# JakubValtar/basisu_rs

Measured on AMD Instinct MI355X. Metric: M 4x4 blocks/s UASTC->BC7 4096x4096, higher is better.
Workload: dtype u8

## Files before the change

### basisu_rs_amd/csrc/bu_hip.hip

```cpp
#include <hip/hip_runtime.h>

#include <stdio.h>
#include <stdlib.h>
#include <string.h>

#include <algorithm>
#include <array>
#include <atomic>
#include <chrono>
#include <future>
#include <iterator>
#include <mutex>
#include <new>
#include <thread>
#include <utility>
#include <vector>

#include "../../include/basisu_hip.h"
#include "bu_basis.hpp"
#include "bu_batch_plan.hpp"
#include "bu_uastc_dispatch.hpp"
#include "bu_etc1s_targets.hpp"
#include "bu_launch_plan.hpp"
#include "bu_rect_plan.hpp"

#include "bu_kernels.hpp"
#include "bu_etc1s_kernels.hpp"
#include "bu_context.hpp"
#include "bu_streams.hpp"
#include "bu_capi_slice.hpp"
#include "bu_capi_file.hpp"
#include "bu_capi_measure.hpp"
#include "bu_multi.hpp"
```

### basisu_rs_amd/csrc/bu_kernels.hpp

```cpp
#pragma once
namespace {

constexpr unsigned bu_lds_front(int target) { return target == 1 ? (unsigned)sizeof(BuBc7Tables) : 0u; }
constexpr unsigned bu_lds_table_bytes(int target) { return bu_lds_front(target) + bu_table_bytes(target); }
template <int WGS, int TARGET>
__device__ __forceinline__ void bu_stage_tables_n(uint4* dst, const BuTablesAll* __restrict__ src)
{
    constexpr BuTableRange R = bu_table_range(TARGET);
    constexpr int F = (int)bu_lds_front(TARGET) / 16;
    const uint4* s = reinterpret_cast<const uint4*>(TARGET == 1 ? reinterpret_cast<const void*>(src) : reinterpret_cast<const void*>(&src->t));
    uint4* d = dst;
    for (int i = threadIdx.x; i < F + (int)(R.hi / 16); i += WGS)
        if (i < F || i >= F + (int)(R.lo / 16)) d[i] = s[i];
    if constexpr (R.lo2 < R.hi2) {
        for (int i = F + R.lo2 / 16 + threadIdx.x; i < F + (int)(R.hi2 / 16); i += WGS) d[i] = s[i];
    }
}

__device__ __forceinline__ void bu_report(unsigned long long* status, unsigned long long block, int st)
{
    if (status) (void)__hip_atomic_fetch_min(status, (block << 8) | (unsigned long long)st, __ATOMIC_RELAXED, __HIP_MEMORY_SCOPE_SYSTEM);
}

typedef unsigned int bu_v4u __attribute__((ext_vector_type(4)));
typedef unsigned int bu_v2u __attribute__((ext_vector_type(2)));
__device__ __forceinline__ uint4 bu_ld_stream(const uint4* p)
{
    const bu_v4u r = __builtin_nontemporal_load(reinterpret_cast<const bu_v4u*>(p));
    return make_uint4(r.x, r.y, r.z, r.w);
}
__device__ __forceinline__ uint4 bu_ld_stream_global(const uint4* p)
{
    typedef const bu_v4u __attribute__((address_space(1))) * bu_global_v4u;
    const bu_v4u r = __builtin_nontemporal_load((bu_global_v4u)p);
    return make_uint4(r.x, r.y, r.z, r.w);
}
typedef bu_v4u __attribute__((address_space(1))) * bu_global_out_v4u;
typedef bu_v2u __attribute__((address_space(1))) * bu_global_out_v2u;
#ifndef BU_ST_MODE
#define BU_ST_MODE 4
#endif
#if BU_ST_MODE == 2
#define BU_ST_BITS " sc1"
#elif BU_ST_MODE == 3
#define BU_ST_BITS " sc0 sc1"
#elif BU_ST_MODE == 4
#define BU_ST_BITS " sc1 nt"
#endif
__device__ __forceinline__ void bu_st_stream(uint4* p, const uint4 v)
{
    bu_v4u r;
    r.x = v.x; r.y = v.y; r.z = v.z; r.w = v.w;
#if BU_ST_MODE == 0
    __builtin_nontemporal_store(r, (bu_global_out_v4u)p);
#elif BU_ST_MODE == 1
    *(bu_global_out_v4u)p = r;
#else
    asm volatile("global_store_dwordx4 %0, %1, off" BU_ST_BITS "\n\ts_nop 1" ::"v"(p), "v"(r) : "memory");
#endif
}
__device__ __forceinline__ void bu_st_stream(uint2* p, const uint2 v)
{
    bu_v2u r;
    r.x = v.x; r.y = v.y;
#if BU_ST_MODE == 1
    *(bu_global_out_v2u)p = r;
#else
    __builtin_nontemporal_store(r, (bu_global_out_v2u)p);
#endif
}

template <int TARGET>
__global__ __launch_bounds__(BU_WG) void bu_uastc_kernel(const uint4* __restrict__ in, void* __restrict__ out, size_t n_blocks,
                                                         unsigned bpr, unsigned long long base, unsigned long long* status,
                                                         const BuTablesAll* __restrict__ tables)
{
    __shared__ uint4 t_store[bu_lds_table_bytes(TARGET) / 16];
    BuTables& T = *reinterpret_cast<BuTables*>(t_store + bu_lds_front(TARGET) / 16);
    const size_t stride = (size_t)gridDim.x * BU_WG;
    size_t idx = (size_t)blockIdx.x * BU_WG + threadIdx.x;
    uint4 v = idx < n_blocks ? bu_ld_stream(in + idx) : make_uint4(0, 0, 0, 0);
    bu_stage_tables_n<BU_WG, TARGET>(t_store, tables);
    __syncthreads();
    while (idx < n_blocks) {
        const size_t next = idx + stride;
        const uint4 vn = next < n_blocks ? in[next] : make_uint4(0, 0, 0, 0);
        BuBlk b;
        b.w[0] = v.x;
        b.w[1] = v.y;
        b.w[2] = v.z;
        b.w[3] = v.w;
        const uint32_t mode = T.mode_lut[v.x & 127u];
        uint32_t o[TARGET == BU_TGT_RGBA ? 16 : 4];
#pragma unroll
        for (int i = 0; i < (TARGET == BU_TGT_RGBA ? 16 : 4); i++) o[i] = 0;
        const int st = bu_block_any<TARGET>(T, mode, b, o);
        if (st) {
            bu_report(status, base + idx, st);
#pragma unroll
            for (int i = 0; i < (TARGET == BU_TGT_RGBA ? 16 : 4); i++) o[i] = 0;
        }
        if constexpr (bu_out_words(TARGET) == 2) {
            reinterpret_cast<uint2*>(out)[idx] = make_uint2(o[0], o[1]);
        } else if constexpr (TARGET == BU_TGT_RGBA) {
            const size_t by = idx / bpr, bx = idx - by * bpr;
            uint4* img = reinterpret_cast<uint4*>(out);
#pragma unroll
            for (int r = 0; r < 4; r++) img[(4 * by + r) * (size_t)bpr + bx] = make_uint4(o[4 * r], o[4 * r + 1], o[4 * r + 2], o[4 * r + 3]);
        } else {
            reinterpret_cast<uint4*>(out)[idx] = make_uint4(o[0], o[1], o[2], o[3]);
        }
        v = vn;
        idx = next;
    }
}

__device__ __forceinline__ uint32_t bu_scan32(uint32_t v)
{
    v += (uint32_t)__builtin_amdgcn_update_dpp(0, (int)v, 0x111, 0xf, 0xf, false);
    v += (uint32_t)__builtin_amdgcn_update_dpp(0, (int)v, 0x112, 0xf, 0xf, false);
    v += (uint32_t)__builtin_amdgcn_update_dpp(0, (int)v, 0x114, 0xf, 0xf, false);
    v += (uint32_t)__builtin_amdgcn_update_dpp(0, (int)v, 0x118, 0xf, 0xf, false);
    v += (uint32_t)__builtin_amdgcn_update_dpp(0, (int)v, 0x142, 0xa, 0xf, false);
    return v;
}

struct BuRunDesc {
    const uint4* in;
    void* out;
    uint64_t base;
    uint32_t n;
    uint32_t vshift;
};
struct BuRunTable {
    BuRunDesc run[BU_MULTI_RUNS];
    uint32_t first_tile[BU_MULTI_RUNS + 32];
};
static_assert(sizeof(BuRunDesc) == 32 && sizeof(BuRunTable) <= 3968, "the run table must fit the 4 KiB of kernel arguments beside the other parameters");
struct BuTileDesc {
    const uint4* in;
    void* out;
    uint32_t first;
    uint32_t n;
    uint64_t base;
    uint32_t width;
};
enum { BU_LAYOUT_STRIP = 0, BU_LAYOUT_RECT = 1, BU_LAYOUT_MULTI = 2,
       BU_LAYOUT_MULTI_WHOLE = 3,
       BU_LAYOUT_RECTS = 4 };
constexpr unsigned BU_TICKET_STRIDE = 32, BU_TICKET_DONE = 8 * BU_TICKET_STRIDE, BU_TICKET_WORDS = 9 * BU_TICKET_STRIDE;
template <int TARGET, int WGS, int BPT, bool PREFETCH, int LAYOUT>
__device__ __forceinline__ void bu_uastc_sorted_body(const uint4* __restrict__ in, void* __restrict__ out, unsigned n_blocks,
                                                     unsigned bpr, unsigned long long base, unsigned long long* status,
                                                     const BuTablesAll* __restrict__ tables, unsigned cus, unsigned tile_rt,
                                                     const BuRunTable* __restrict__ runs, unsigned* __restrict__ ticket = nullptr,
                                                     const BuRectTable* __restrict__ rects = nullptr)
{
    if (cus != 0) {
        constexpr bool ROT = TARGET == BU_TGT_BC7 || TARGET == BU_TGT_ASTC;
        if (blockIdx.x >= 3 * cus) __builtin_amdgcn_s_setprio(ROT ? 1 : 3);
        else if (blockIdx.x >= 2 * cus) __builtin_amdgcn_s_setprio(2);
        else if (blockIdx.x >= cus) __builtin_amdgcn_s_setprio(ROT ? 3 : 1);
    }
    constexpr int BU_WG = WGS, BU_BPT = BPT, BU_TILE = WGS * BPT;
    __shared__ uint4 t_store[bu_lds_table_bytes(TARGET) / 16];
    BuTables& T = *reinterpret_cast<BuTables*>(t_store + bu_lds_front(TARGET) / 16);
    constexpr bool RECT = LAYOUT == BU_LAYOUT_RECT, MULTI = LAYOUT == BU_LAYOUT_MULTI || LAYOUT == BU_LAYOUT_MULTI_WHOLE;
    constexpr bool WHOLE = RECT || LAYOUT == BU_LAYOUT_MULTI_WHOLE;
    constexpr bool RECTS = LAYOUT == BU_LAYOUT_RECTS;
    static_assert(!RECTS || (BU_TILE == (int)BU_RECTS_TILE && PREFETCH), "the host numbers 1024-block tiles of rectangles; one compiled shape");
    constexpr uint32_t RECTS_ROW_BYTES = bu_rect_row_bytes(TARGET), RECTS_ROWS = bu_rect_rows_per_block(TARGET);
    constexpr bool BU_ALIAS = TARGET == BU_TGT_RGBA;
    static_assert(!BU_ALIAS || bu_lds_table_bytes(TARGET) + 4 * BU_TILE * 16 + BU_TILE + 1536 <= 80 * 1024,
                  "the RGBA32 workgroup no longer fits twice per CU: shrink BuTables or stage it per target in LDS too");
    __shared__ uint4 sblk_store[BU_ALIAS ? 1 : BU_TILE];
    __shared__ uint4 sout[BU_ALIAS ? 4 * BU_TILE : 1];
    uint4* const sblk = BU_ALIAS ? sout : sblk_store;
    constexpr bool INBLOCK = TARGET == BU_TGT_BC7 || TARGET == BU_TGT_ASTC;
    __shared__ uint8_t sst[INBLOCK ? 16 : BU_TILE];
    __shared__ uint32_t cnt[2][32], next_chunk[2];
    const unsigned tid = threadIdx.x, lane = tid & 63u;
    constexpr bool DYN_TILE = bu_dyn_tile(TARGET, BU_TILE) && LAYOUT != BU_LAYOUT_RECT;
    const unsigned tile_blocks = DYN_TILE ? tile_rt : (unsigned)BU_TILE;
    const unsigned n_tiles = (n_blocks + tile_blocks - 1) / tile_blocks;
    auto in_tile = [&](unsigned l) { return !DYN_TILE || l < tile_blocks; };
    static_assert(!RECT || BU_TILE % BU_RECT_W == 0, "rectangular tiles are BU_RECT_W blocks wide and of fixed size");
    const unsigned tpr = RECT ? bpr / BU_RECT_W : 1u;
    auto tile_xy = [&](unsigned t, unsigned& ty, unsigned& tx) {
        ty = (unsigned)(((unsigned long long)t * tile_rt) >> 32);
        tx = t - ty * tpr;
    };
    auto gidx = [&](unsigned t, unsigned l) {
        if constexpr (RECT) {
            unsigned ty, tx;
            tile_xy(t, ty, tx);
            return ((unsigned)(BU_TILE / BU_RECT_W) * ty + l / BU_RECT_W) * bpr + BU_RECT_W * tx + (l % BU_RECT_W);
        } else {
            return t * tile_blocks + l;
        }
    };
    auto has_block = [&](uint32_t k) { return WHOLE || k < 20u; };
    unsigned tile = blockIdx.x;
    __shared__ uint32_t s_next_tile[2];
    uint32_t my_draw = 0;
    unsigned* const my_counter = ticket ? ticket + (blockIdx.x & 7u) * BU_TICKET_STRIDE : nullptr;
    auto tile_of_draw = [&](uint32_t d) { return gridDim.x + 8u * d + (blockIdx.x & 7u); };
    if (ticket && tid == 0) my_draw = atomicAdd(my_counter, 1u);
    BuTileDesc td = {in, out, 0u, 0u, base, 0u}, tl = td;
    constexpr bool RUNS_IN_LDS = (MULTI || RECTS) && PREFETCH;
    __shared__ uint4 s_runs[RUNS_IN_LDS ? (RECTS ? sizeof(BuRectTable) : sizeof(BuRunTable)) / 16 : 1];
    const BuRunTable* R = runs;
    const BuRectTable* Q = rects;
    if constexpr (RUNS_IN_LDS && RECTS) {
        for (unsigned i = tid; i < sizeof(BuRectTable) / 16; i += WGS) s_runs[i] = reinterpret_cast<const uint4*>(rects)[i];
    } else if constexpr (RUNS_IN_LDS) {
        static_assert(sizeof(BuRunTable) % 16 == 0, "copied in 16-byte pieces");
        for (unsigned i = tid; i < sizeof(BuRunTable) / 16; i += WGS) s_runs[i] = reinterpret_cast<const uint4*>(runs)[i];
    }
    auto uni32 = [](uint32_t x) { return (uint32_t)__builtin_amdgcn_readfirstlane((int)x); };
    auto uni64 = [&](uint64_t x) { return (uint64_t)uni32((uint32_t)x) | ((uint64_t)uni32((uint32_t)(x >> 32)) << 32); };
    auto desc_of = [&](unsigned t, BuTileDesc& d) {
        if constexpr (MULTI) {
            if (t < n_tiles) {
                uint32_t r = 0;
#pragma unroll
                for (unsigned c = 0; c < BU_MULTI_RUNS + 32; c += 64) {
                    const uint32_t cnt = (uint32_t)__popcll(__ballot(R->first_tile[c + lane] <= t));
                    if (cnt) r = c + cnt - 1u;
                }
                r = (uint32_t)__builtin_amdgcn_readfirstlane((int)r);
                const BuRunDesc rv = R->run[r];
                const BuRunDesc rd = {reinterpret_cast<const uint4*>(uni64(reinterpret_cast<uint64_t>(rv.in))), reinterpret_cast<void*>(uni64(reinterpret_cast<uint64_t>(rv.out))),
                                      uni64(rv.base), uni32(rv.n), uni32(rv.vshift)};
                const uint32_t lt = t - uni32(R->first_tile[r]);
                if (rd.vshift != BU_RUN_STRIPS) {
                    const uint32_t ty = lt >> rd.vshift, tx = lt & ((1u << rd.vshift) - 1u), width = (uint32_t)BU_RECT_W << rd.vshift;
                    d = BuTileDesc{rd.in, rd.out, (uint32_t)(BU_TILE / BU_RECT_W) * ty * width + (uint32_t)BU_RECT_W * tx, (uint32_t)BU_TILE, rd.base, width};
                } else {
                    const uint32_t first = lt * (uint32_t)BU_TILE, left = rd.n - first;
                    d = BuTileDesc{rd.in, rd.out, first, left < (uint32_t)BU_TILE ? left : (uint32_t)BU_TILE, rd.base, 0u};
                }
            }
        }
    };
    BuRectTile qd = {}, ql = {};
    auto rect_of = [&](unsigned t, BuRectTile& d) {
        if constexpr (RECTS) {
            if (t < n_tiles) {
                static_assert(BU_RECT_JOBS == 64, "one first-tile number per lane");
                const uint32_t r = uni32((uint32_t)__popcll(__ballot(Q->first_tile[lane] <= t)) - 1u);
                const BuRectDesc jv = Q->job[r];
                const BuRectDesc jd = {uni64(jv.in), uni64(jv.out), uni64(jv.pitch), uni64(jv.base), uni32(jv.in_bpr), uni32(jv.w), uni32(jv.h), uni32(jv.tpr)};
                d = bu_rect_tile(jd, t - uni32(Q->first_tile[r]), RECTS_ROW_BYTES, RECTS_ROWS);
            }
        }
    };
    desc_of(tile, td);
    tl = td;
    rect_of(tile, qd);
    ql = qd;
    auto run_idx = [&](const BuTileDesc& d, unsigned l) { return d.first + ((WHOLE || d.width) ? (l / BU_RECT_W) * d.width + (l % BU_RECT_W) : l); };
    auto blk_src = [&](unsigned t, unsigned l) { return RECTS ? reinterpret_cast<const uint4*>(bu_rect_src(ql, l)) : MULTI ? tl.in + run_idx(tl, l) : in + gidx(t, l); };
    auto ld_blk = [&](unsigned t, unsigned l) { return (MULTI || RECTS) ? bu_ld_stream_global(blk_src(t, l)) : bu_ld_stream(blk_src(t, l)); };
    auto blk_valid = [&](unsigned t, unsigned l) {
        if constexpr (RECTS) return t < n_tiles && bu_rect_has(ql, l);
        else if constexpr (MULTI) return t < n_tiles && (WHOLE || l < tl.n);
        else return RECT ? t < n_tiles : (t < n_tiles && gidx(t, l) < n_blocks && in_tile(l));
    };
    constexpr BuTableRange TR = bu_table_range(TARGET);
    constexpr bool SPLIT = bu_lds_table_bytes(TARGET) > 16384;
    constexpr int TF = (int)bu_lds_front(TARGET) / 16, TV1 = (int)(TR.hi - TR.lo) / 16, TV2 = TR.lo2 < TR.hi2 ? (int)(TR.hi2 - TR.lo2) / 16 : 0;
    constexpr int TVT = TF + TV1 + TV2, TVN = (TVT + WGS - 1) / WGS;
    const uint4* const tsrc = reinterpret_cast<const uint4*>(TARGET == BU_TGT_BC7 ? reinterpret_cast<const void*>(tables) : reinterpret_cast<const void*>(&tables->t));
    auto tdst = [&](int i) { return i < TF ? i : (i < TF + TV1 ? (int)(TR.lo / 16) + i : TF + (int)(TR.lo2 / 16) + (i - TF - TV1)); };
    uint4 tv[TVN];
    if constexpr (!SPLIT) {
#pragma unroll
        for (int k = 0; k < TVN; k++) {
            const int i = k * WGS + (int)tid;
            tv[k] = i < TVT ? tsrc[tdst(i)] : make_uint4(0, 0, 0, 0);
        }
    }
    uint4 v[BU_BPT];
#pragma unroll
    for (int j = 0; j < BU_BPT; j++)
        v[j] = (RECT || blk_valid(tile, j * BU_WG + tid)) ? ld_blk(tile, j * BU_WG + tid) : make_uint4(0, 0, 0, 0);
    if constexpr (!SPLIT) {
#pragma unroll
        for (int k = 0; k < TVN; k++) {
            const int i = k * WGS + (int)tid;
            if (i < TVT) t_store[tdst(i)] = tv[k];
        }
    } else {
#pragma unroll
        for (int k = 0; k < TVN; k++) {
            const int i = k * WGS + (int)tid;
            tv[k] = i < TVT ? tsrc[tdst(i)] : make_uint4(0, 0, 0, 0);
        }
        static_assert(offsetof(BuTables, key_lut) % 4 == 0 && sizeof(T.key_lut[0]) == 128, "the target's key_lut is staged as 32 dwords");
        if (tid < 32) reinterpret_cast<uint32_t*>(T.key_lut[bu_cost_row(TARGET)])[tid] = reinterpret_cast<const uint32_t*>(tables->t.key_lut[bu_cost_row(TARGET)])[tid];
    }
    bool tables_staged = !SPLIT;
    if (tid < 64) (&cnt[0][0])[tid] = 0;
    if (tid < 2) next_chunk[tid] = 0;
    __syncthreads();
    if constexpr (RUNS_IN_LDS && RECTS) Q = reinterpret_cast<const BuRectTable*>(s_runs);
    else if constexpr (RUNS_IN_LDS) R = reinterpret_cast<const BuRunTable*>(s_runs);
    unsigned par = 0;
    unsigned next_of_loop = 0;
    constexpr bool STORES_LAST = PREFETCH && MULTI && (TARGET == BU_TGT_BC7 || (TARGET == BU_TGT_ASTC && WGS == 256 && WHOLE));
    auto key_of = [&](const BuTileDesc& d, unsigned l, uint32_t x) { return (WHOLE || l < d.n) ? (uint32_t)T.key_lut[bu_cost_row(TARGET)][x & 127u] : 31u; };
    uint32_t next_key[STORES_LAST ? BU_BPT : 1];
    uint32_t drawn_tile = 0;
    if constexpr (STORES_LAST) {
        if (tile < n_tiles) {
#pragma unroll
            for (int j = 0; j < BU_BPT; j++) next_key[j] = key_of(td, j * BU_WG + tid, v[j].x);
        }
        if (ticket && tid == 0) drawn_tile = tile_of_draw(my_draw);
        __builtin_amdgcn_s_waitcnt(0x0F70);
    }
    for (; tile < n_tiles; tile = next_of_loop, par ^= 1u) {
        [[maybe_unused]] const unsigned tbase = tile * tile_blocks;
        uint32_t key[BU_BPT], pos[BU_BPT];
        bool uniform = true;
#pragma unroll
        for (int j = 0; j < BU_BPT; j++) {
            if constexpr (STORES_LAST) {
                key[j] = next_key[j];
            } else {
                const bool valid = WHOLE || (RECTS ? bu_rect_has(qd, (unsigned)(j * BU_WG) + tid) : MULTI ? (unsigned)(j * BU_WG) + tid < td.n : (tbase + j * BU_WG + tid < n_blocks && in_tile(j * BU_WG + tid)));
                key[j] = valid ? T.key_lut[bu_cost_row(TARGET)][v[j].x & 127u] : 31u;
            }
            uniform = uniform && (__ballot(key[j] == (uint32_t)__builtin_amdgcn_readfirstlane(key[j])) == ~0ull) && has_block(key[j]);
        }
        if (uniform) {
            uint32_t lead[BU_BPT];
#pragma unroll
            for (int j = 0; j < BU_BPT; j++) lead[j] = lane == 0 ? atomicAdd(&cnt[par][key[j]], 64u) : 0u;
#pragma unroll
            for (int j = 0; j < BU_BPT; j++) pos[j] = (uint32_t)__builtin_amdgcn_readfirstlane(lead[j]) + lane;
        } else {
#pragma unroll
            for (int j = 0; j < BU_BPT; j++) pos[j] = atomicAdd(&cnt[par][key[j]], 1u);
        }
        if (ticket && tid == 0) s_next_tile[par] = STORES_LAST ? drawn_tile : tile_of_draw(my_draw);
        if (!tables_staged) {
#pragma unroll
            for (int k = 0; k < TVN; k++) {
                const int i = k * WGS + (int)tid;
                if (i < TVT) t_store[tdst(i)] = tv[k];
            }
            tables_staged = true;
        }
        __syncthreads();
        const uint32_t run_c = lane < 20u ? cnt[par][lane] : 0u;
        const uint32_t run_pk = run_c | (((run_c + 63u) >> 6) << 16);
        const uint32_t run_incl = bu_scan32(run_pk), run_excl = run_incl - run_pk;
        const uint32_t nc = (uint32_t)__builtin_amdgcn_readlane((int)run_incl, 31) >> 16;
        if (tid < 32) cnt[par ^ 1u][tid] = 0;
        if (tid == 0) next_chunk[par ^ 1u] = 0;
        uint32_t dest[BU_BPT];
#pragma unroll
        for (int j = 0; j < BU_BPT; j++) {
            const uint32_t st = (uint32_t)__builtin_amdgcn_ds_bpermute((int)(key[j] << 2), (int)run_excl) & 0xFFFFu;
            dest[j] = has_block(key[j]) ? st + pos[j] : 0u;
            if (has_block(key[j])) sblk[dest[j]] = v[j];
        }
        const unsigned ntile = ticket ? (unsigned)__builtin_amdgcn_readfirstlane((int)s_next_tile[par]) : tile + gridDim.x;
        next_of_loop = ntile;
        uint4 vn[BU_BPT];
        if constexpr (PREFETCH) {
            desc_of(ntile, tl);
            rect_of(ntile, ql);
#pragma unroll
            for (int j = 0; j < BU_BPT; j++) {
                vn[j] = blk_valid(ntile, j * BU_WG + tid) ? ld_blk(ntile, j * BU_WG + tid) : make_uint4(0, 0, 0, 0);
            }
        }
        if (ticket && tid == 0 && ntile < n_tiles) my_draw = atomicAdd(my_counter, 1u);
        __syncthreads();
        uint32_t c_next = 0;
        if (lane == 0) c_next = atomicAdd(&next_chunk[par], 1u);
        for (;;) {
            const uint32_t c = __builtin_amdgcn_readfirstlane(c_next);
            if (c >= nc) break;
            if (lane == 0) c_next = atomicAdd(&next_chunk[par], 1u);
            const uint32_t r = (uint32_t)__builtin_ctzll(__ballot((run_incl >> 16) > c));
            const uint32_t r_pk = (uint32_t)__builtin_amdgcn_readlane((int)run_pk, (int)r), r_ex = (uint32_t)__builtin_amdgcn_readlane((int)run_excl, (int)r);
            const uint32_t k64 = (c - (r_ex >> 16)) << 6;
            const uint32_t s0 = (r_ex & 0xFFFFu) + k64, left = (r_pk & 0xFFFFu) - k64, count = left < 64u ? left : 64u;
            const bool active = lane < count;
            const uint32_t slot = s0 + (active ? lane : 0u);
            const uint4 bv = sblk[slot];
            BuBlk b;
            b.w[0] = bv.x;
            b.w[1] = bv.y;
            b.w[2] = bv.z;
            b.w[3] = bv.w;
            constexpr int NO = TARGET == BU_TGT_RGBA ? 16 : 4;
            uint32_t o[NO];
#pragma unroll
            for (int i = 0; i < NO; i++) o[i] = 0;
            int st = BU_ST_BAD_MODE;
            if (active) {
                switch (r) {
#define BU_CASE(k) \
    case k: st = bu_block_mode<TARGET, BU_COST_ORDER[bu_cost_row(TARGET)][k]>(T, b, o); break;
                    BU_CASE(0) BU_CASE(1) BU_CASE(2) BU_CASE(3) BU_CASE(4) BU_CASE(5) BU_CASE(6) BU_CASE(7) BU_CASE(8) BU_CASE(9)
                    BU_CASE(10) BU_CASE(11) BU_CASE(12) BU_CASE(13) BU_CASE(14) BU_CASE(15) BU_CASE(16) BU_CASE(17) BU_CASE(18)
#undef BU_CASE
                default: break;
                }
                if constexpr (TARGET == BU_TGT_RGBA) {
#pragma unroll
                    for (int r2 = 0; r2 < 4; r2++) sout[r2 * BU_TILE + slot] = make_uint4(o[4 * r2], o[4 * r2 + 1], o[4 * r2 + 2], o[4 * r2 + 3]);
                    sst[slot] = (uint8_t)st;
                } else if constexpr (INBLOCK) {
                    sblk[slot] = make_uint4(o[0], o[1], o[2], o[3] | (uint32_t)st);
                } else {
                    sblk[slot] = make_uint4(o[0], o[1], o[2], o[3]);
                    sst[slot] = (uint8_t)st;
                }
            }
        }
        __syncthreads();
        if constexpr (STORES_LAST) {
            uint4 r[BU_BPT];
            bool has[BU_BPT];
            auto out_idx = [&](int j) { return run_idx(td, j * BU_WG + tid); };
#pragma unroll
            for (int j = 0; j < BU_BPT; j++) {
                has[j] = has_block(key[j]);
                if (has[j]) {
                    r[j] = sblk[dest[j]];
                    if ((r[j].x & 0xFFu) == 0u) {
                        bu_report(status, td.base + out_idx(j), (int)r[j].w);
                        r[j].w = 0;
                    }
                }
            }
#pragma unroll
            for (int j = 0; j < BU_BPT; j++) next_key[j] = key_of(tl, j * BU_WG + tid, vn[j].x);
            drawn_tile = tile_of_draw(my_draw);
            asm volatile("" : "+v"(drawn_tile));
#pragma unroll
            for (int j = 0; j < BU_BPT; j++)
                if (has[j]) bu_st_stream(reinterpret_cast<uint4*>(td.out) + out_idx(j), r[j]);
        } else {
#pragma unroll
        for (int j = 0; j < BU_BPT; j++) {
            if constexpr (RECTS) {
                if (has_block(key[j])) {
                    const unsigned l = j * BU_WG + tid;
                    const unsigned long long blk = qd.base + bu_rect_idx(qd, l);
                    const uint64_t dst = bu_rect_dst(qd, l, RECTS_ROW_BYTES, RECTS_ROWS);
                    if constexpr (INBLOCK) {
                        uint4 r = sblk[dest[j]];
                        if ((r.x & 0xFFu) == 0u) {
                            bu_report(status, blk, (int)r.w);
                            r.w = 0;
                        }
                        bu_st_stream(reinterpret_cast<uint4*>(dst), r);
                    } else {
                        const uint32_t st = sst[dest[j]];
                        if (st) bu_report(status, blk, (int)st);
                        if constexpr (TARGET == BU_TGT_RGBA) {
#pragma unroll
                            for (int r = 0; r < 4; r++) bu_st_stream(reinterpret_cast<uint4*>(dst + (uint64_t)r * qd.pitch), sout[r * BU_TILE + dest[j]]);
                        } else {
                            const uint4 r = sblk[dest[j]];
                            if constexpr (bu_out_words(TARGET) == 2) bu_st_stream(reinterpret_cast<uint2*>(dst), make_uint2(r.x, r.y));
                            else bu_st_stream(reinterpret_cast<uint4*>(dst), r);
                        }
                    }
                }
                continue;
            }
            if (has_block(key[j])) {
                const unsigned idx = MULTI ? run_idx(td, j * BU_WG + tid) : gidx(tile, j * BU_WG + tid);
                void* const out = td.out;
                const unsigned long long base = td.base;
                if constexpr (INBLOCK) {
                    uint4 r = sblk[dest[j]];
                    if ((r.x & 0xFFu) == 0u) {
                        bu_report(status, base + idx, (int)r.w);
                        r.w = 0;
                    }
                    bu_st_stream(reinterpret_cast<uint4*>(out) + idx, r);
                    continue;
                }
                const uint32_t st = sst[dest[j]];
                if (st) bu_report(status, base + idx, (int)st);
                if constexpr (TARGET == BU_TGT_RGBA) {
                    unsigned by, bx;
                    if constexpr (RECT) {
                        const unsigned l = j * BU_WG + tid;
                        unsigned ty, tx;
                        tile_xy(tile, ty, tx);
                        by = (unsigned)(BU_TILE / BU_RECT_W) * ty + l / BU_RECT_W;
                        bx = BU_RECT_W * tx + (l % BU_RECT_W);
                    } else {
                        by = idx / bpr;
                        bx = idx - by * bpr;
                    }
                    uint4* img = reinterpret_cast<uint4*>(out);
#pragma unroll
                    for (int r = 0; r < 4; r++) bu_st_stream(img + (size_t)((4 * by + r) * bpr + bx), sout[r * BU_TILE + dest[j]]);
                } else {
                    const uint4 r = sblk[dest[j]];
                    if constexpr (bu_out_words(TARGET) == 2) bu_st_stream(reinterpret_cast<uint2*>(out) + idx, make_uint2(r.x, r.y));
                    else bu_st_stream(reinterpret_cast<uint4*>(out) + idx, r);
                }
            }
        }
        }
        if constexpr (PREFETCH) {
#pragma unroll
            for (int j = 0; j < BU_BPT; j++) v[j] = vn[j];
            td = tl;
            qd = ql;
        } else {
            desc_of(ntile, tl);
            td = tl;
            rect_of(ntile, ql);
            qd = ql;
#pragma unroll
            for (int j = 0; j < BU_BPT; j++) v[j] = blk_valid(ntile, j * BU_WG + tid) ? ld_blk(ntile, j * BU_WG + tid) : make_uint4(0, 0, 0, 0);
        }
    }
    if (ticket && tid == 0) {
        if (atomicAdd(ticket + BU_TICKET_DONE, 1u) == gridDim.x - 1u) {
            for (unsigned k = 0; k < 8; k++) atomicExch(ticket + k * BU_TICKET_STRIDE, 0u);
            atomicExch(ticket + BU_TICKET_DONE, 0u);
        }
    }
}

template <int TARGET, int WGS, int BPT, int MINW, bool PREFETCH, int LAYOUT>
__global__ __launch_bounds__(WGS, MINW) void bu_uastc_sorted_kernel(const uint4* __restrict__ in, void* __restrict__ out, unsigned n_blocks,
                                                                unsigned bpr, unsigned long long base, unsigned long long* status,
                                                                const BuTablesAll* __restrict__ tables, unsigned cus, unsigned tile_rt,
                                                                unsigned* __restrict__ ticket)
{
    static_assert(LAYOUT != BU_LAYOUT_MULTI && LAYOUT != BU_LAYOUT_MULTI_WHOLE, "several runs per launch: bu_uastc_multi_kernel");
    bu_uastc_sorted_body<TARGET, WGS, BPT, PREFETCH, LAYOUT>(in, out, n_blocks, bpr, base, status, tables, cus, tile_rt, nullptr, ticket);
}

constexpr bool bu_multi_etc_2048(int target, int tile) { return bu_etc_family(target) && tile == 2048; }
template <int TARGET, int WGS, int BPT, bool PREFETCH = false, bool WHOLE = false>
__global__ __launch_bounds__(WGS, (TARGET == BU_TGT_ASTC && WGS == 512) ? 8 : bu_multi_etc_2048(TARGET, WGS * BPT) ? 4 : 1) void bu_uastc_multi_kernel(
    const BuRunTable table, unsigned n_tiles, unsigned bpr, unsigned long long* status, const BuTablesAll* __restrict__ tables, unsigned* __restrict__ ticket)
{
    static_assert(WGS * BPT == 1024 || bu_multi_etc_2048(TARGET, WGS * BPT), "the host numbers 1024-block tiles (ETC1 / ETC2 large batches: 2048-block ones)");
    static_assert(sizeof(BuRunTable) + 40 <= 4096, "the run table and the other arguments share the 4 KiB of kernel arguments");
    bu_uastc_sorted_body<TARGET, WGS, BPT, PREFETCH, WHOLE ? BU_LAYOUT_MULTI_WHOLE : BU_LAYOUT_MULTI>(nullptr, nullptr, n_tiles * (unsigned)(WGS * BPT), bpr, 0ull, status, tables, 0u,
                                                                                                        (unsigned)(WGS * BPT), &table, ticket);
}

template <int TARGET>
__global__ __launch_bounds__(512) void bu_uastc_rects_kernel(const BuRectTable table, unsigned n_tiles, unsigned long long* status, const BuTablesAll* __restrict__ tables)
{
    static_assert(sizeof(BuRectTable) + 24 <= 4096, "the job table and the other arguments share the 4 KiB of kernel arguments");
    bu_uastc_sorted_body<TARGET, 512, 2, true, BU_LAYOUT_RECTS>(nullptr, nullptr, n_tiles * BU_RECTS_TILE, 0u, 0ull, status, tables, 0u, BU_RECTS_TILE, nullptr, nullptr, &table);
}

__global__ void bu_status_reset_kernel(unsigned long long* words, unsigned n)
{
    for (unsigned i = threadIdx.x; i < n; i += blockDim.x) words[i] = ~0ull;
}

struct BuCrcTables {
    uint16_t t[4][256];
    uint16_t pw[256];
};
constexpr unsigned BU_CRC_PIECE = 65536;

__device__ __forceinline__ uint32_t bu_crc_gf_mul(uint32_t a, uint32_t b)
{
    uint32_t r = 0;
#pragma unroll
// ... 65 lines not shown
```

### basisu_rs_amd/csrc/bu_launch_plan.hpp

```cpp
#pragma once
#include <stddef.h>
#include <stdint.h>

#include <vector>

#include "bu_batch_plan.hpp"
#include "bu_uastc_dispatch.hpp"

constexpr int BU_WG = 256;
constexpr int BU_SORT_MIN_BLOCKS = 8;
constexpr bool bu_dyn_tile(int target, int tile) { return bu_etc_family(target) && tile == 4096; }
constexpr unsigned BU_RECT_W = 64;
constexpr unsigned BU_MULTI_RUNS = 96;
constexpr uint32_t BU_RUN_STRIPS = 0xFFFFFFFFu;
constexpr unsigned BU_TICKET_MIN_GRID = 8;

inline unsigned bu_grid_for(size_t n_blocks, unsigned cu_count)
{
    size_t wgs = (n_blocks + BU_WG - 1) / BU_WG;
    const size_t cap = (size_t)cu_count * 8;
    if (wgs > cap) wgs = cap;
    if (wgs == 0) wgs = 1;
    return (unsigned)wgs;
}

constexpr unsigned BU_ZEROCOPY_GRID = 64;

inline size_t bu_balanced_tile(size_t max_tile, size_t n_blocks, size_t slots, bool dynamic)
{
    if (!dynamic || slots == 0) return max_tile;
    const size_t per_slot = (n_blocks + slots - 1) / slots, rounds = (per_slot + max_tile - 1) / max_tile;
    size_t t = ((per_slot + rounds - 1) / rounds + 63) & ~(size_t)63;
    return t < 64 ? 64 : (t > max_tile ? max_tile : t);
}

struct BuShape {
    int wgs, bpt, minw;
    bool prefetch, rect;
    int per_cu;
    constexpr size_t tile() const { return (size_t)wgs * bpt; }
};
enum { BU_POLICY_EXCLUSIVE = 0, BU_POLICY_SHARED = 1, BU_POLICY_AUTO = 2,
       BU_POLICY_SHARED_FEW = 3 };
constexpr BuShape BuBigShape(int target, int policy)
{
    if (target == BU_TGT_BC7 || target == BU_TGT_ASTC)
        return policy == BU_POLICY_SHARED ? BuShape{256, 4, 1, true, true, 2}
                                          : BuShape{512, 2, target == BU_TGT_ASTC ? 8 : 1, true, true, 4};
    return policy == BU_POLICY_SHARED ? BuShape{512, 4, 4, target == BU_TGT_ETC1, true, 1} : BuShape{1024, 4, 1, true, true, 1};
}
constexpr bool bu_big_from_one_tile_per_cu(int target) { return target == BU_TGT_BC7 || target == BU_TGT_ASTC; }
constexpr BuShape BuOneTileShape(int target) { return BuShape{1024, 1, 1, false, target == BU_TGT_BC7 || target == BU_TGT_ASTC, 1}; }
constexpr BuShape BuEtcMidShape{512, 2, 1, false, false, 3};
constexpr BuShape BuZeroCopyShape{256, 4, 1, true, false, 1};
constexpr int BU_HOST_TILE = 1024;

struct BuSortedKey { int target, wgs, bpt, minw; bool prefetch, rect; };
constexpr BuSortedKey BU_SORTED_KERNELS[] = {
    {BU_TGT_BC7, 1024, 1, 1, false, false}, {BU_TGT_BC7, 1024, 1, 1, false, true}, {BU_TGT_BC7, 512, 2, 1, true, false}, {BU_TGT_BC7, 512, 2, 1, true, true},
    {BU_TGT_BC7, 256, 4, 1, true, false}, {BU_TGT_BC7, 256, 4, 1, true, true}, {BU_TGT_BC7, 512, 2, 1, false, false},
    {BU_TGT_ASTC, 1024, 1, 1, false, false}, {BU_TGT_ASTC, 1024, 1, 1, false, true}, {BU_TGT_ASTC, 512, 2, 8, true, false}, {BU_TGT_ASTC, 512, 2, 8, true, true},
    {BU_TGT_ASTC, 256, 4, 1, true, false}, {BU_TGT_ASTC, 256, 4, 1, true, true}, {BU_TGT_ASTC, 512, 2, 1, false, false},
    {BU_TGT_ETC1, 1024, 1, 1, false, false}, {BU_TGT_ETC1, 512, 2, 1, false, false}, {BU_TGT_ETC1, 1024, 4, 1, true, false}, {BU_TGT_ETC1, 1024, 4, 1, true, true},
    {BU_TGT_ETC1, 512, 4, 4, true, false}, {BU_TGT_ETC1, 512, 4, 4, true, true}, {BU_TGT_ETC1, 256, 4, 1, true, false}, {BU_TGT_ETC1, 256, 4, 1, true, true},
    {BU_TGT_ETC2, 1024, 1, 1, false, false}, {BU_TGT_ETC2, 512, 2, 1, false, false}, {BU_TGT_ETC2, 1024, 4, 1, true, false}, {BU_TGT_ETC2, 1024, 4, 1, true, true},
    {BU_TGT_ETC2, 512, 4, 4, false, false}, {BU_TGT_ETC2, 512, 4, 4, false, true}, {BU_TGT_ETC2, 256, 4, 1, true, false}, {BU_TGT_ETC2, 256, 4, 1, true, true},
    {BU_TGT_RGBA, 1024, 1, 1, true, false}, {BU_TGT_RGBA, 1024, 1, 1, true, true}, {BU_TGT_RGBA, 512, 2, 1, true, false}, {BU_TGT_RGBA, 512, 2, 1, true, true},
// ... 73 lines not shown
            const size_t slots = (size_t)cu_count * S.per_cu;
            const size_t tile_rt = bu_balanced_tile(S.tile(), nb, slots, bu_dyn_tile(target, (int)S.tile()));
            const size_t big_tiles = (nb + tile_rt - 1) / tile_rt;
            const unsigned cus = (priorities && (big_tiles <= slots || big_tiles % slots == 0)) ? cu_count : 0u;
            const bool ticket = priorities && bu_ticket_target(target) && big_tiles >= BU_TICKET_MIN_WALK * slots;
            go(S, big_tiles < slots ? big_tiles : slots, cus, tile_rt, ticket);
        };
        if (target == BU_TGT_RGBA) {
            const size_t cap = grid_cap ? (size_t)grid_cap : (size_t)cu_count * (policy == BU_POLICY_SHARED ? 1 : 2);
            const size_t grid = tiles < cap ? tiles : cap;
            const unsigned cus = (policy != BU_POLICY_SHARED && tiles >= 2 * grid) ? cu_count : 0u;
            const bool ticket = policy != BU_POLICY_SHARED && tiles >= BU_TICKET_MIN_WALK * grid;
            const bool wide = grid_cap == 0 && nb <= ((size_t)3 << 20);
            go(wide ? BuShape{1024, 1, 1, true, true, 2} : BuShape{512, 2, 1, true, true, 2}, grid, cus, BU_HOST_TILE, ticket);
        } else if (grid_cap) {
            go(BuZeroCopyShape, tiles < grid_cap ? tiles : grid_cap, cu_count, BuZeroCopyShape.tile(), false);
        } else if (nb <= (size_t)BU_HOST_TILE * cu_count) {
            go(BuOneTileShape(target), tiles, cu_count, BU_HOST_TILE, false);
        } else if (bu_big_from_one_tile_per_cu(target) || nb > (size_t)3 * BU_HOST_TILE * cu_count) {
            const BuShape shared = BuBigShape(target, BU_POLICY_SHARED);
            if (etc && nb >= ((size_t)1 << 20))
                go(shared, (nb + shared.tile() - 1) / shared.tile(), 0u, shared.tile(), false);
            else if (policy == BU_POLICY_SHARED_FEW && bu_big_from_one_tile_per_cu(target))
                go_big(BuShape{shared.wgs, shared.bpt, shared.minw, shared.prefetch, shared.rect, 4}, false);
            else if (policy == BU_POLICY_SHARED || policy == BU_POLICY_SHARED_FEW) go_big(shared, false);
            else if (target == BU_TGT_ASTC && nb >= ((size_t)1 << 21))
                go_big(BuShape{256, 4, 1, true, true, 5}, true);
            else go_big(BuBigShape(target, BU_POLICY_EXCLUSIVE), true);
        } else {
            go(BuEtcMidShape, tiles, cu_count, BU_HOST_TILE, false);
        }
    }
}

struct BuRunEntry { size_t run, offset, n; uint32_t vshift, first_tile; };
enum { BU_MULTI_ETC_2048 = 0, BU_MULTI_ONE_TILE = 1, BU_MULTI_WHOLE = 2, BU_MULTI_PERSIST = 3 };
struct BuRunsLaunch {
    size_t plain_run = SIZE_MAX;
    BuRunEntry entries[BU_MULTI_RUNS];
    size_t k = 0, n_tiles = 0;
    unsigned tile = 1024;
    bool all_whole = true;
    bool needs_policy = false;
    int kernel = BU_MULTI_PERSIST;
    unsigned grid = 0, block = 0;
    bool wants_ticket = false;
};

inline void bu_plan_runs(int kernel_target, const BuRun* runs, size_t n_runs, size_t blocks_per_row, unsigned cu_count, std::vector<BuRunsLaunch>& out)
{
    const int target = bu_shape_target(kernel_target);
    out.clear();
    const bool rect_target = target == BU_TGT_BC7 || target == BU_TGT_ASTC || target == BU_TGT_RGBA;
    const size_t real = (blocks_per_row >= 128 && (blocks_per_row & (blocks_per_row - 1)) == 0 && blocks_per_row <= ((size_t)1 << 20)) ? blocks_per_row : 0;
    const size_t virt = target == BU_TGT_RGBA ? 0 : 1;
    const size_t pitches[5] = {real, virt * 1024, virt * 2048, virt * 512, virt * 256};
    auto shift_of = [](size_t v) {
        uint32_t sh = 0;
        while (((size_t)BU_RECT_W << sh) < v) sh++;
        return sh;
    };
    for (size_t r0 = 0; r0 < n_runs;) {
        BuRunsLaunch l;
        if (target == BU_TGT_ETC1 || target == BU_TGT_ETC2) {
            size_t total = 0, tiles2 = 0;
            for (size_t i = r0; i < n_runs && i < r0 + BU_MULTI_RUNS; i++) {
                total += runs[i].n;
                tiles2 += (runs[i].n + 2047) / 2048;
            }
            if (total >= ((size_t)1 << 20) && tiles2 * 2048 <= total + total / 8) l.tile = 2048;
        }
        auto emit = [&](size_t run, size_t offset, size_t n, uint32_t vshift) {
            l.all_whole = l.all_whole && vshift != BU_RUN_STRIPS;
            l.entries[l.k++] = BuRunEntry{run, offset, n, vshift, (uint32_t)l.n_tiles};
            l.n_tiles += (n + l.tile - 1) / l.tile;
        };
        size_t used = 0;
        for (; r0 + used < n_runs && l.k < BU_MULTI_RUNS; used++) {
            const size_t ri = r0 + used, n = runs[ri].n;
            const size_t t = (n + l.tile - 1) / l.tile;
            if (l.n_tiles + t + 1 >= (((size_t)1 << 32) / l.tile)) break;
            size_t whole_pitch = 0, prefix_pitch = 0;
            if (rect_target) {
                for (const size_t v : pitches)
                    if (v && n % (16 * v) == 0) {
                        whole_pitch = v;
                        break;
                    }
                if (!whole_pitch && target == BU_TGT_RGBA && l.k + 2 <= BU_MULTI_RUNS)
                    for (const size_t v : pitches)
                        if (v && n >= 8 * 16 * v) {
                            prefix_pitch = v;
                            break;
                        }
            }
            if (whole_pitch) {
                emit(ri, 0, n, shift_of(whole_pitch));
            } else if (prefix_pitch) {
                const size_t prefix = n / (16 * prefix_pitch) * (16 * prefix_pitch);
                emit(ri, 0, prefix, shift_of(prefix_pitch));
                emit(ri, prefix, n - prefix, BU_RUN_STRIPS);
            } else {
                emit(ri, 0, n, BU_RUN_STRIPS);
            }
        }
        if (used <= 1) {
            out.emplace_back().plain_run = r0++;
            continue;
        }
        l.needs_policy = !(l.tile == 1024 && l.n_tiles <= (size_t)cu_count);
        out.push_back(l);
        r0 += used;
    }
}

// ... 15 lines not shown
```

Measured before the change: 189,800.

## Cache run lookup and precompute 32-bit lane offsets in multi-run kernel

The multi-run kernel now keeps a cursor on the current run and skips the ballot search over the run table when the next tile falls in the same run. Per-lane byte offsets are computed once per tile width and reused. Loads and stores use a uniform 64-bit base plus a 32-bit per-lane offset, so the store can use the SGPR-base addressing form. This is meant to cut per-tile descriptor work and per-block 64-bit address arithmetic, at the cost of more registers and a new constraint that offsets fit in 32 bits (large RGBA pitches fall back to plain runs).

```diff
diff --git a/basisu_rs_amd/csrc/bu_hip.hip b/basisu_rs_amd/csrc/bu_hip.hip
--- a/basisu_rs_amd/csrc/bu_hip.hip
+++ b/basisu_rs_amd/csrc/bu_hip.hip
@@ -23,6 +23,7 @@
 #include "bu_etc1s_targets.hpp"
 #include "bu_launch_plan.hpp"
 #include "bu_rect_plan.hpp"
+#include "bu_multi_addr.hpp"
 
 #include "bu_kernels.hpp"
 #include "bu_etc1s_kernels.hpp"
diff --git a/basisu_rs_amd/csrc/bu_kernels.hpp b/basisu_rs_amd/csrc/bu_kernels.hpp
--- a/basisu_rs_amd/csrc/bu_kernels.hpp
+++ b/basisu_rs_amd/csrc/bu_kernels.hpp
@@ -33,6 +33,13 @@
 {
     typedef const bu_v4u __attribute__((address_space(1))) * bu_global_v4u;
     const bu_v4u r = __builtin_nontemporal_load((bu_global_v4u)p);
+    return make_uint4(r.x, r.y, r.z, r.w);
+}
+typedef const char __attribute__((address_space(1))) * bu_global_bytes;
+__device__ __forceinline__ uint4 bu_ld_stream_global(uint64_t base, uint32_t off)
+{
+    typedef const bu_v4u __attribute__((address_space(1))) * bu_global_v4u;
+    const bu_v4u r = __builtin_nontemporal_load((bu_global_v4u)((bu_global_bytes)base + off));
     return make_uint4(r.x, r.y, r.z, r.w);
 }
 typedef bu_v4u __attribute__((address_space(1))) * bu_global_out_v4u;
@@ -67,6 +74,29 @@
     *(bu_global_out_v2u)p = r;
 #else
     __builtin_nontemporal_store(r, (bu_global_out_v2u)p);
+#endif
+}
+typedef char __attribute__((address_space(1))) * bu_global_out_bytes;
+__device__ __forceinline__ void bu_st_stream(uint64_t base, uint32_t off, const uint4 v)
+{
+    bu_v4u r;
+    r.x = v.x; r.y = v.y; r.z = v.z; r.w = v.w;
+#if BU_ST_MODE == 0
+    __builtin_nontemporal_store(r, (bu_global_out_v4u)((bu_global_out_bytes)base + off));
+#elif BU_ST_MODE == 1
+    *(bu_global_out_v4u)((bu_global_out_bytes)base + off) = r;
+#else
+    asm volatile("global_store_dwordx4 %0, %1, %2" BU_ST_BITS "\n\ts_nop 1" ::"v"(off), "v"(r), "s"(base) : "memory");
+#endif
+}
+__device__ __forceinline__ void bu_st_stream(uint64_t base, uint32_t off, const uint2 v)
+{
+    bu_v2u r;
+    r.x = v.x; r.y = v.y;
+#if BU_ST_MODE == 1
+    *(bu_global_out_v2u)((bu_global_out_bytes)base + off) = r;
+#else
+    __builtin_nontemporal_store(r, (bu_global_out_v2u)((bu_global_out_bytes)base + off));
 #endif
 }
 
@@ -145,6 +175,19 @@
     uint64_t base;
     uint32_t width;
 };
+template <bool MULTI, int BPT>
+struct BuMultiWalk {
+    BuMultiTile d = {}, l = {};
+    uint32_t off[BPT] = {};
+    uint32_t off_width = 0xFFFFFFFFu;
+    BuRunCursor cur = bu_no_run();
+};
+template <int BPT>
+struct BuMultiWalk<false, BPT> {};
+template <int BPT>
+__device__ __forceinline__ uint32_t bu_walk_n(const BuMultiWalk<true, BPT>& w) { return w.d.n; }
+template <int BPT>
+__device__ __forceinline__ uint32_t bu_walk_n(const BuMultiWalk<false, BPT>&) { return 0u; }
 enum { BU_LAYOUT_STRIP = 0, BU_LAYOUT_RECT = 1, BU_LAYOUT_MULTI = 2,
        BU_LAYOUT_MULTI_WHOLE = 3,
        BU_LAYOUT_RECTS = 4 };
@@ -207,6 +250,8 @@
     auto tile_of_draw = [&](uint32_t d) { return gridDim.x + 8u * d + (blockIdx.x & 7u); };
     if (ticket && tid == 0) my_draw = atomicAdd(my_counter, 1u);
     BuTileDesc td = {in, out, 0u, 0u, base, 0u}, tl = td;
+    BuMultiWalk<MULTI, BPT> mw;
+    constexpr uint32_t OUT_BYTES = TARGET == BU_TGT_RGBA ? 16u : (uint32_t)bu_out_words(TARGET) * 4u;
     constexpr bool RUNS_IN_LDS = (MULTI || RECTS) && PREFETCH;
     __shared__ uint4 s_runs[RUNS_IN_LDS ? (RECTS ? sizeof(BuRectTable) : sizeof(BuRunTable)) / 16 : 1];
     const BuRunTable* R = runs;
@@ -219,26 +264,28 @@
     }
     auto uni32 = [](uint32_t x) { return (uint32_t)__builtin_amdgcn_readfirstlane((int)x); };
     auto uni64 = [&](uint64_t x) { return (uint64_t)uni32((uint32_t)x) | ((uint64_t)uni32((uint32_t)(x >> 32)) << 32); };
-    auto desc_of = [&](unsigned t, BuTileDesc& d) {
+    auto desc_of = [&](unsigned t, BuMultiTile& d) {
         if constexpr (MULTI) {
             if (t < n_tiles) {
-                uint32_t r = 0;
-#pragma unroll
-                for (unsigned c = 0; c < BU_MULTI_RUNS + 32; c += 64) {
-                    const uint32_t cnt = (uint32_t)__popcll(__ballot(R->first_tile[c + lane] <= t));
-                    if (cnt) r = c + cnt - 1u;
-                }
-                r = (uint32_t)__builtin_amdgcn_readfirstlane((int)r);
-                const BuRunDesc rv = R->run[r];
-                const BuRunDesc rd = {reinterpret_cast<const uint4*>(uni64(reinterpret_cast<uint64_t>(rv.in))), reinterpret_cast<void*>(uni64(reinterpret_cast<uint64_t>(rv.out))),
-                                      uni64(rv.base), uni32(rv.n), uni32(rv.vshift)};
-                const uint32_t lt = t - uni32(R->first_tile[r]);
-                if (rd.vshift != BU_RUN_STRIPS) {
-                    const uint32_t ty = lt >> rd.vshift, tx = lt & ((1u << rd.vshift) - 1u), width = (uint32_t)BU_RECT_W << rd.vshift;
-                    d = BuTileDesc{rd.in, rd.out, (uint32_t)(BU_TILE / BU_RECT_W) * ty * width + (uint32_t)BU_RECT_W * tx, (uint32_t)BU_TILE, rd.base, width};
-                } else {
-                    const uint32_t first = lt * (uint32_t)BU_TILE, left = rd.n - first;
-                    d = BuTileDesc{rd.in, rd.out, first, left < (uint32_t)BU_TILE ? left : (uint32_t)BU_TILE, rd.base, 0u};
+                if (!bu_cursor_holds(mw.cur, t)) {
+                    uint32_t r = 0;
+                    uint32_t ln = lane;
+                    asm volatile("" : "+v"(ln));
+#pragma unroll
+                    for (unsigned c = 0; c < BU_MULTI_RUNS + 32; c += 64) {
+                        const uint32_t cnt = (uint32_t)__popcll(__ballot(R->first_tile[c + ln] <= t));
+                        if (cnt) r = c + cnt - 1u;
+                    }
+                    r = (uint32_t)__builtin_amdgcn_readfirstlane((int)r);
+                    const BuRunDesc rv = R->run[r];
+                    const BuRunRec rd = {uni64(reinterpret_cast<uint64_t>(rv.in)), uni64(reinterpret_cast<uint64_t>(rv.out)), uni64(rv.base), uni32(rv.n), uni32(rv.vshift)};
+                    mw.cur = bu_run_cursor(rd, uni32(R->first_tile[r]), (uint32_t)BU_TILE);
+                }
+                d = bu_tile_of(mw.cur, t, (uint32_t)BU_TILE, OUT_BYTES, TARGET == BU_TGT_RGBA ? bpr : 0u);
+                if (d.width != mw.off_width) {
+                    mw.off_width = d.width;
+#pragma unroll
+                    for (int j = 0; j < BPT; j++) mw.off[j] = bu_lane_off(WHOLE, d.width, (unsigned)(j * WGS) + tid);
                 }
             }
         }
@@ -255,16 +302,30 @@
             }
         }
     };
-    desc_of(tile, td);
+    if constexpr (MULTI) desc_of(tile, mw.d);
+    if constexpr (MULTI) mw.l = mw.d;
     tl = td;
     rect_of(tile, qd);
     ql = qd;
-    auto run_idx = [&](const BuTileDesc& d, unsigned l) { return d.first + ((WHOLE || d.width) ? (l / BU_RECT_W) * d.width + (l % BU_RECT_W) : l); };
-    auto blk_src = [&](unsigned t, unsigned l) { return RECTS ? reinterpret_cast<const uint4*>(bu_rect_src(ql, l)) : MULTI ? tl.in + run_idx(tl, l) : in + gidx(t, l); };
-    auto ld_blk = [&](unsigned t, unsigned l) { return (MULTI || RECTS) ? bu_ld_stream_global(blk_src(t, l)) : bu_ld_stream(blk_src(t, l)); };
+    auto blk_src = [&](unsigned t, unsigned l) { return RECTS ? reinterpret_cast<const uint4*>(bu_rect_src(ql, l)) : in + gidx(t, l); };
+    auto ld_one = [&](unsigned t, unsigned l) { return RECTS ? bu_ld_stream_global(blk_src(t, l)) : bu_ld_stream(blk_src(t, l)); };
+    auto ld_blk = [&](unsigned t, unsigned l, int j) {
+        if constexpr (MULTI) return bu_ld_stream_global(mw.l.in, mw.off[j]);
+        else return ld_one(t, l);
+    };
+    auto store_offsets = [&](uint32_t (&so)[MULTI ? BPT : 1]) {
+        if constexpr (MULTI) {
+#pragma unroll
+            for (int j = 0; j < BPT; j++) so[j] = mw.off[j];
+            if (mw.d.width != mw.off_width) {
+#pragma unroll
+                for (int j = 0; j < BPT; j++) so[j] = bu_lane_off(WHOLE, mw.d.width, (unsigned)(j * WGS) + tid);
+            }
+        }
+    };
     auto blk_valid = [&](unsigned t, unsigned l) {
         if constexpr (RECTS) return t < n_tiles && bu_rect_has(ql, l);
-        else if constexpr (MULTI) return t < n_tiles && (WHOLE || l < tl.n);
+        else if constexpr (MULTI) return t < n_tiles && (WHOLE || l < mw.l.n);
         else return RECT ? t < n_tiles : (t < n_tiles && gidx(t, l) < n_blocks && in_tile(l));
     };
     constexpr BuTableRange TR = bu_table_range(TARGET);
@@ -284,7 +345,7 @@
     uint4 v[BU_BPT];
 #pragma unroll
     for (int j = 0; j < BU_BPT; j++)
-        v[j] = (RECT || blk_valid(tile, j * BU_WG + tid)) ? ld_blk(tile, j * BU_WG + tid) : make_uint4(0, 0, 0, 0);
+        v[j] = (RECT || blk_valid(tile, j * BU_WG + tid)) ? ld_blk(tile, j * BU_WG + tid, j) : make_uint4(0, 0, 0, 0);
     if constexpr (!SPLIT) {
 #pragma unroll
         for (int k = 0; k < TVN; k++) {
@@ -309,13 +370,13 @@
     unsigned par = 0;
     unsigned next_of_loop = 0;
     constexpr bool STORES_LAST = PREFETCH && MULTI && (TARGET == BU_TGT_BC7 || (TARGET == BU_TGT_ASTC && WGS == 256 && WHOLE));
-    auto key_of = [&](const BuTileDesc& d, unsigned l, uint32_t x) { return (WHOLE || l < d.n) ? (uint32_t)T.key_lut[bu_cost_row(TARGET)][x & 127u] : 31u; };
+    auto key_of = [&](const BuMultiTile& d, unsigned l, uint32_t x) { return (WHOLE || l < d.n) ? (uint32_t)T.key_lut[bu_cost_row(TARGET)][x & 127u] : 31u; };
     uint32_t next_key[STORES_LAST ? BU_BPT : 1];
     uint32_t drawn_tile = 0;
     if constexpr (STORES_LAST) {
         if (tile < n_tiles) {
 #pragma unroll
-            for (int j = 0; j < BU_BPT; j++) next_key[j] = key_of(td, j * BU_WG + tid, v[j].x);
+            for (int j = 0; j < BU_BPT; j++) next_key[j] = key_of(mw.d, j * BU_WG + tid, v[j].x);
         }
         if (ticket && tid == 0) drawn_tile = tile_of_draw(my_draw);
         __builtin_amdgcn_s_waitcnt(0x0F70);
@@ -329,7 +390,7 @@
             if constexpr (STORES_LAST) {
                 key[j] = next_key[j];
             } else {
-                const bool valid = WHOLE || (RECTS ? bu_rect_has(qd, (unsigned)(j * BU_WG) + tid) : MULTI ? (unsigned)(j * BU_WG) + tid < td.n : (tbase + j * BU_WG + tid < n_blocks && in_tile(j * BU_WG + tid)));
+                const bool valid = WHOLE || (RECTS ? bu_rect_has(qd, (unsigned)(j * BU_WG) + tid) : MULTI ? (unsigned)(j * BU_WG) + tid < bu_walk_n(mw) : (tbase + j * BU_WG + tid < n_blocks && in_tile(j * BU_WG + tid)));
                 key[j] = valid ? T.key_lut[bu_cost_row(TARGET)][v[j].x & 127u] : 31u;
             }
             uniform = uniform && (__ballot(key[j] == (uint32_t)__builtin_amdgcn_readfirstlane(key[j])) == ~0ull) && has_block(key[j]);
@@ -371,11 +432,21 @@
         next_of_loop = ntile;
         uint4 vn[BU_BPT];
         if constexpr (PREFETCH) {
-            desc_of(ntile, tl);
+            if constexpr (MULTI) desc_of(ntile, mw.l);
             rect_of(ntile, ql);
-#pragma unroll
-            for (int j = 0; j < BU_BPT; j++) {
-                vn[j] = blk_valid(ntile, j * BU_WG + tid) ? ld_blk(ntile, j * BU_WG + tid) : make_uint4(0, 0, 0, 0);
+            if constexpr (MULTI && WHOLE) {
+                if (ntile < n_tiles) {
+#pragma unroll
+                    for (int j = 0; j < BU_BPT; j++) vn[j] = ld_blk(ntile, j * BU_WG + tid, j);
+                } else {
+#pragma unroll
+                    for (int j = 0; j < BU_BPT; j++) vn[j] = make_uint4(0, 0, 0, 0);
+                }
+            } else {
+#pragma unroll
+                for (int j = 0; j < BU_BPT; j++) {
+                    vn[j] = blk_valid(ntile, j * BU_WG + tid) ? ld_blk(ntile, j * BU_WG + tid, j) : make_uint4(0, 0, 0, 0);
+                }
             }
         }
         if (ticket && tid == 0 && ntile < n_tiles) my_draw = atomicAdd(my_counter, 1u);
@@ -428,26 +499,29 @@
         if constexpr (STORES_LAST) {
             uint4 r[BU_BPT];
             bool has[BU_BPT];
-            auto out_idx = [&](int j) { return run_idx(td, j * BU_WG + tid); };
+            uint32_t so[BU_BPT];
+            store_offsets(so);
 #pragma unroll
             for (int j = 0; j < BU_BPT; j++) {
                 has[j] = has_block(key[j]);
                 if (has[j]) {
                     r[j] = sblk[dest[j]];
                     if ((r[j].x & 0xFFu) == 0u) {
-                        bu_report(status, td.base + out_idx(j), (int)r[j].w);
+                        bu_report(status, mw.d.base + bu_lane_block(mw.d, so[j]), (int)r[j].w);
                         r[j].w = 0;
                     }
                 }
             }
 #pragma unroll
-            for (int j = 0; j < BU_BPT; j++) next_key[j] = key_of(tl, j * BU_WG + tid, vn[j].x);
+            for (int j = 0; j < BU_BPT; j++) next_key[j] = key_of(mw.l, j * BU_WG + tid, vn[j].x);
             drawn_tile = tile_of_draw(my_draw);
             asm volatile("" : "+v"(drawn_tile));
 #pragma unroll
             for (int j = 0; j < BU_BPT; j++)
-                if (has[j]) bu_st_stream(reinterpret_cast<uint4*>(td.out) + out_idx(j), r[j]);
+                if (has[j]) bu_st_stream(mw.d.out, so[j], r[j]);
         } else {
+        [[maybe_unused]] uint32_t so[MULTI ? BU_BPT : 1];
+        store_offsets(so);
 #pragma unroll
         for (int j = 0; j < BU_BPT; j++) {
             if constexpr (RECTS) {
@@ -477,8 +551,34 @@
                 }
                 continue;
             }
+            if constexpr (MULTI) {
+                if (has_block(key[j])) {
+                    const uint32_t lo = so[j];
+                    if constexpr (INBLOCK) {
+                        uint4 r = sblk[dest[j]];
+                        if ((r.x & 0xFFu) == 0u) {
+                            bu_report(status, mw.d.base + bu_lane_block(mw.d, lo), (int)r.w);
+                            r.w = 0;
+                        }
+                        bu_st_stream(mw.d.out, lo, r);
+                    } else {
+                        const uint32_t st = sst[dest[j]];
+                        if (st) bu_report(status, mw.d.base + bu_lane_block(mw.d, lo), (int)st);
+                        if constexpr (TARGET == BU_TGT_RGBA) {
+                            const uint32_t row0 = bu_lane_off_rgba(mw.d, lo, bpr);
+#pragma unroll
+                            for (int r = 0; r < 4; r++) bu_st_stream(mw.d.out, row0 + (uint32_t)r * bpr * 16u, sout[r * BU_TILE + dest[j]]);
+                        } else {
+                            const uint4 r = sblk[dest[j]];
+                            if constexpr (bu_out_words(TARGET) == 2) bu_st_stream(mw.d.out, lo >> 1, make_uint2(r.x, r.y));
+                            else bu_st_stream(mw.d.out, lo, r);
+                        }
+                    }
+                }
+                continue;
+            }
             if (has_block(key[j])) {
-                const unsigned idx = MULTI ? run_idx(td, j * BU_WG + tid) : gidx(tile, j * BU_WG + tid);
+                const unsigned idx = gidx(tile, j * BU_WG + tid);
                 void* const out = td.out;
                 const unsigned long long base = td.base;
                 if constexpr (INBLOCK) {
@@ -519,14 +619,16 @@
 #pragma unroll
             for (int j = 0; j < BU_BPT; j++) v[j] = vn[j];
             td = tl;
+            if constexpr (MULTI) mw.d = mw.l;
             qd = ql;
         } else {
-            desc_of(ntile, tl);
+            if constexpr (MULTI) desc_of(ntile, mw.l);
+            if constexpr (MULTI) mw.d = mw.l;
             td = tl;
             rect_of(ntile, ql);
             qd = ql;
 #pragma unroll
-            for (int j = 0; j < BU_BPT; j++) v[j] = blk_valid(ntile, j * BU_WG + tid) ? ld_blk(ntile, j * BU_WG + tid) : make_uint4(0, 0, 0, 0);
+            for (int j = 0; j < BU_BPT; j++) v[j] = blk_valid(ntile, j * BU_WG + tid) ? ld_blk(ntile, j * BU_WG + tid, j) : make_uint4(0, 0, 0, 0);
         }
     }
     if (ticket && tid == 0) {
diff --git a/basisu_rs_amd/csrc/bu_launch_plan.hpp b/basisu_rs_amd/csrc/bu_launch_plan.hpp
--- a/basisu_rs_amd/csrc/bu_launch_plan.hpp
+++ b/basisu_rs_amd/csrc/bu_launch_plan.hpp
@@ -13,6 +13,8 @@
 constexpr unsigned BU_RECT_W = 64;
 constexpr unsigned BU_MULTI_RUNS = 96;
 constexpr uint32_t BU_RUN_STRIPS = 0xFFFFFFFFu;
+constexpr size_t BU_MULTI_MAX_WIDTH = (size_t)1 << 20;
+constexpr size_t BU_MULTI_RGBA_MAX_BPR = (size_t)1 << 24;
 constexpr unsigned BU_TICKET_MIN_GRID = 8;
 
 inline unsigned bu_grid_for(size_t n_blocks, unsigned cu_count)
@@ -192,7 +194,7 @@
     const int target = bu_shape_target(kernel_target);
     out.clear();
     const bool rect_target = target == BU_TGT_BC7 || target == BU_TGT_ASTC || target == BU_TGT_RGBA;
-    const size_t real = (blocks_per_row >= 128 && (blocks_per_row & (blocks_per_row - 1)) == 0 && blocks_per_row <= ((size_t)1 << 20)) ? blocks_per_row : 0;
+    const size_t real = (blocks_per_row >= 128 && (blocks_per_row & (blocks_per_row - 1)) == 0 && blocks_per_row <= BU_MULTI_MAX_WIDTH) ? blocks_per_row : 0;
     const size_t virt = target == BU_TGT_RGBA ? 0 : 1;
     const size_t pitches[5] = {real, virt * 1024, virt * 2048, virt * 512, virt * 256};
     auto shift_of = [](size_t v) {
@@ -201,6 +203,10 @@
         return sh;
     };
     for (size_t r0 = 0; r0 < n_runs;) {
+        if (target == BU_TGT_RGBA && blocks_per_row > BU_MULTI_RGBA_MAX_BPR) {
+            out.emplace_back().plain_run = r0++;
+            continue;
+        }
         BuRunsLaunch l;
         if (target == BU_TGT_ETC1 || target == BU_TGT_ETC2) {
             size_t total = 0, tiles2 = 0;
diff --git a/basisu_rs_amd/csrc/bu_multi_addr.hpp b/basisu_rs_amd/csrc/bu_multi_addr.hpp
--- /dev/null
+++ b/basisu_rs_amd/csrc/bu_multi_addr.hpp
@@ -0,0 +1,76 @@
+#pragma once
+#include <stdint.h>
+
+#include "bu_launch_plan.hpp"
+
+struct BuRunRec {
+    uint64_t in, out, base;
+    uint32_t n;
+    uint32_t vshift;
+};
+struct BuRunCursor {
+    BuRunRec run;
+    uint32_t first_tile, n_tiles;
+};
+struct BuMultiTile {
+    uint64_t in;
+    uint64_t out;
+    uint64_t base;
+    uint32_t first;
+    uint32_t n;
+    uint32_t width;
+    uint32_t bx0;
+};
+
+BU_DEV BuRunCursor bu_no_run() { return BuRunCursor{BuRunRec{0, 0, 0, 0u, BU_RUN_STRIPS}, 0u, 0u}; }
+BU_DEV BuRunCursor bu_run_cursor(const BuRunRec& r, uint32_t first_tile, uint32_t tile) { return BuRunCursor{r, first_tile, r.n / tile + (r.n % tile ? 1u : 0u)}; }
+BU_DEV bool bu_cursor_holds(const BuRunCursor& c, uint32_t t) { return t - c.first_tile < c.n_tiles; }
+
+BU_DEV BuMultiTile bu_tile_of(const BuRunCursor& c, uint32_t t, uint32_t tile, uint32_t out_bytes, uint32_t rgba_bpr)
+{
+    const BuRunRec& r = c.run;
+    const uint32_t lt = t - c.first_tile;
+    BuMultiTile d;
+    if (r.vshift != BU_RUN_STRIPS) {
+        const uint32_t ty = lt >> r.vshift, tx = lt & ((1u << r.vshift) - 1u);
+        d.width = (uint32_t)BU_RECT_W << r.vshift;
+        d.first = (tile / (uint32_t)BU_RECT_W) * ty * d.width + (uint32_t)BU_RECT_W * tx;
+        d.n = tile;
+    } else {
+        d.width = 0u;
+        d.first = lt * tile;
+        d.n = r.n - d.first < tile ? r.n - d.first : tile;
+    }
+    d.in = r.in + (uint64_t)d.first * 16u;
+    d.base = r.base;
+    if (rgba_bpr) {
+        const uint32_t by0 = d.first / rgba_bpr;
+        d.bx0 = d.first - by0 * rgba_bpr;
+        d.out = r.out + (uint64_t)by0 * rgba_bpr * 64u;
+    } else {
+        d.bx0 = 0u;
+        d.out = r.out + (uint64_t)d.first * out_bytes;
+    }
+    return d;
+}
+
+BU_DEV uint32_t bu_lane_off(bool whole, uint32_t width, uint32_t l)
+{
+    return ((whole || width) ? (l / (uint32_t)BU_RECT_W) * width + (l % (uint32_t)BU_RECT_W) : l) * 16u;
+}
+static_assert((uint64_t)((2048 / BU_RECT_W - 1) * (uint64_t)BU_MULTI_MAX_WIDTH + BU_RECT_W - 1) * 16u < ((uint64_t)1 << 32), "a lane offset fits 32 bits");
+BU_DEV uint64_t bu_lane_block(const BuMultiTile& d, uint32_t off) { return (uint64_t)d.first + (off >> 4); }
+
+BU_DEV uint32_t bu_lane_off_rgba(const BuMultiTile& d, uint32_t off, uint32_t bpr)
+{
+    const uint32_t c = d.bx0 + (off >> 4), dy = c / bpr;
+    return (3u * dy * bpr + c) * 16u;
+}
+static_assert((7 * (uint64_t)BU_MULTI_RGBA_MAX_BPR + 4 * ((2048 / BU_RECT_W) * (uint64_t)BU_MULTI_MAX_WIDTH)) * 16u < ((uint64_t)1 << 32), "an RGBA32 lane offset fits 32 bits");
+
+inline uint32_t bu_run_of_tile(const uint32_t* first_tile, uint32_t entries, uint32_t t)
+{
+    uint32_t cnt = 0;
+    for (uint32_t i = 0; i < entries; i++) cnt += first_tile[i] <= t;
+    return cnt - 1u;
+}
```

New measurement: 192,100 (median of 6 runs). 1.2% higher.
